# ERGO-Code/ipx

Measured on AMD Instinct MI355X. Metric: kkt_solves_per_sec, higher is better.
Workload: dtype f64; 1 GPU; C3 synthetic LP m=1000000 n=2000000 8 nnz/col (nnz=16000000), KKTSolverDiag::Solve = diag-precond CR to tol=0.3*sqrt(mu), scaling spread s=1; rows of AI partitioned over 1 GPU(s); errflag=0

## Files before the change

### ipx_amd/csrc/api.hip

```cpp

#include <algorithm>
#include <map>
#include <thread>

#include "context.hpp"

namespace ipxk {

static thread_local std::string g_last_error;
void set_last_error(const std::string& msg) { g_last_error = msg; }

Context::~Context() {
    if (split) destroy_split(split);
    if (split_spare) destroy_split(split_spare);
    if (prepare_host) destroy_prepare_host(prepare_host);
    if (lu) destroy_lu(lu);
    if (maxvol) destroy_maxvol(maxvol);
    if (nmat) destroy_nmatrix(nmat);
    comm_destroy(this);
    if (h_state) (void)hipHostFree(h_state);
    if (h_cycle_done) (void)hipHostFree(h_cycle_done);
    if (ev_a) (void)hipEventDestroy(ev_a);
    if (ev_b) (void)hipEventDestroy(ev_b);
    for (hipEvent_t e : ev_window) (void)hipEventDestroy(e);
// ... 1198 lines not shown
        IPXK_REQUIRE(c && info && (which == 0 || which == 1), "bad argument");
        const GatherMatrix& M = which == 0 ? c->Acols : c->Arows;
        for (int i = 0; i < 40; i++) info[i] = 0;
        const SpmvLayout L = M.layout;
        info[0] = M.tile_base() != SpmvLayout::phased; info[1] = L == SpmvLayout::sorted; info[2] = L == SpmvLayout::sortedfused; info[3] = M.nlong;
        info[4] = M.sliced.built; info[5] = M.sliced.R; info[6] = M.sliced.nslices; info[7] = M.sliced.nrb;
        info[8] = M.sliced.nrows_pad; info[9] = M.sliced.max_tile;
        { double d = M.sliced.dominant_fraction; memcpy(&info[10], &d, sizeof d); }
        info[11] = M.sorted.built; info[12] = M.sorted.nslices; info[13] = M.sorted.nsub; info[14] = M.sorted.nrb;
        info[15] = M.sorted.RB; info[16] = M.sorted.nrows_pad; info[17] = M.sorted.max_sub; info[18] = M.sorted.slice_elems;
        info[19] = M.sorted.fused; info[20] = M.nnz;
        info[21] = M.P; info[22] = M.G; info[23] = (ipxint)M.RT * 1000000 + (ipxint)M.Q * 1000 + 0;
        info[24] = L == SpmvLayout::acc; info[25] = M.acc.built; info[26] = M.acc.nslices; info[27] = M.acc.nrb; info[28] = M.acc.RB;
        info[29] = M.acc.nrows_pad; info[30] = M.acc.slice_elems; info[31] = M.acc.nbatches; info[32] = M.acc.deferred;
        info[33] = L == SpmvLayout::accfused; info[34] = M.accf.built; info[35] = M.accf.nrb; info[36] = M.accf.RB; info[37] = M.accf.nbatches;
        info[38] = L == SpmvLayout::plain;
        if (create_ms) for (int i = 0; i < 4; i++) create_ms[i] = c->create_ms[i];
    });
}
int ipxk_layout_array(ipxk_context* c, int which, int array, void* out, ipxint cap, ipxint* nbytes) {
    return guarded([&] {
        IPXK_REQUIRE(c && nbytes && (which == 0 || which == 1), "bad argument");
        bind_device(c);
        const GatherMatrix& M = which == 0 ? c->Acols : c->Arows;
        const void* src = nullptr;
        size_t bytes = 0;
        const size_t ntiles = (size_t)M.sliced.nrb * M.sliced.nslices, nsubs = (size_t)M.sorted.nrb * std::max(M.sorted.nslices, 1) * std::max(M.sorted.nsub, 1);
        const size_t nz = (size_t)M.nnz;
        switch (array) {
            case 0: src = M.sliced.tile_ptr.get(); bytes = M.sliced.built ? (ntiles + 1) * 4 : 0; break;
            case 1: src = M.sliced.cnt.get(); bytes = M.sliced.built ? ntiles * M.sliced.R : 0; break;
// ... 4 lines not shown
            case 6: src = M.sorted.pack.get(); bytes = M.sorted.built ? nz * 4 : 0; break;
            case 7: src = M.sorted.val.get(); bytes = M.sorted.built ? nz * 8 : 0; break;
            case 8: src = c->pl_Tp.get(); bytes = ((size_t)c->m + 1) * 4; break;
            case 9: src = c->pl_Ti.get(); bytes = (size_t)c->nnz * 4; break;
            case 10: src = c->pl_Tx.get(); bytes = (size_t)c->nnz * 8; break;
            case 11: src = M.acc.tile_batch.get(); bytes = M.acc.built ? ((size_t)M.acc.nrb * M.acc.nslices + 1) * 4 : 0; break;
            case 12: src = M.acc.bptr.get(); bytes = M.acc.built ? ((size_t)M.acc.nbatches + 1) * 4 : 0; break;
            case 13: src = M.acc.pack.get(); bytes = M.acc.built ? nz * 4 : 0; break;
            case 14: src = M.acc.val.get(); bytes = M.acc.built ? nz * 8 : 0; break;
            case 15: src = M.accf.tile_batch.get(); bytes = M.accf.built ? ((size_t)M.accf.nrb + 1) * 4 : 0; break;
            case 16: src = M.accf.bptr.get(); bytes = M.accf.built ? ((size_t)M.accf.nbatches + 1) * 4 : 0; break;
            case 17: src = M.accf.pack.get(); bytes = M.accf.built ? nz * 4 : 0; break;
            case 18: src = M.accf.val.get(); bytes = M.accf.built ? nz * 8 : 0; break;
            case 19: src = M.accf.xmin.get(); bytes = M.accf.built ? (size_t)M.accf.nrb * 4 : 0; break;
            case 20: src = M.sorted.xmin.get(); bytes = M.sorted.built && M.sorted.fused ? (size_t)M.sorted.nrb * 4 : 0; break;
            default: IPXK_REQUIRE(false, "unknown array");
        }
        if (M.nlong > 0 && (array < 8 || array > 10)) bytes = 0;
        *nbytes = (ipxint)bytes;
        const size_t ncopy = std::min<size_t>(bytes, cap > 0 ? (size_t)cap : 0);
        if (out && ncopy > 0) staged_d2h(out, src, ncopy, c->stream);
    });
}

ipxint ipxk_normal_apply_bytes(const ipxk_context* c) {
    if (!c) return 0;
    const ipxint wi = 4;
    return 2 * c->nnz * (wi + 8) + (c->n + c->m + 2) * wi + 8 * (3 * c->n + 4 * c->m);
}

// ... 50 lines not shown
```

### ipx_amd/csrc/context.hpp

```cpp
#pragma once

#include "internal.hpp"
#include "device_utils.hpp"

struct ncclComm;

namespace ipxk {

constexpr int kPartialStride = kMaxPartials + 8;

enum PartialSlot {
    kPartRes0 = 0,
    kPartRes1,
    kPartPdot,
    kPartCdot,
    kPartRsdot,
    kPartScratch,
    kNumPartialSlots
};

struct Reordered {
    bool active = false;
    int levels = 0;
    int components = 0;
// ... 136 lines not shown
void device_transpose(Tmp& T, DevBuf<int>& colof, int64_t n, int64_t m, int64_t nz, const int* Ap, const int* Ai, const double* Ax, int* Tp,
                      int* Ti, double* Tx, hipStream_t s);

bool device_strip_long_rows(LayoutScratch& S, GatherMatrix& G, int nrows, const int* dptr, const int* didx, const double* dval,
                            DevBuf<int>& sptr, DevBuf<int>& sidx, DevBuf<double>& sval, int64_t* nnz_short, hipStream_t s);
bool device_build_sliced(LayoutScratch& S, SlicedMatrix& out, int nrows, int ncols, int64_t nnz, const int* dptr, const int* didx,
                         const double* dval, hipStream_t s, int ns_request = 0);
bool device_build_sorted_fused(LayoutScratch& S, SortedMatrix& out, int nrows, int ncols, int64_t nnz, const int* dptr, const int* didx,
                               const double* dval, hipStream_t s);
bool device_build_acc_fused(LayoutScratch& S, AccMatrix& out, int nrows, int ncols, int64_t nnz, const int* dptr, const int* didx,
                            const double* dval, hipStream_t s);
bool device_build_sorted(LayoutScratch& S, SortedMatrix& out, const SlicedMatrix& sliced, int nrows, int ncols, int64_t nnz, const int* dptr,
                         const int* didx, const double* dval, hipStream_t s);
bool device_build_acc(LayoutScratch& S, AccMatrix& out, const SlicedMatrix& sliced, int nrows, int ncols, int64_t nnz, const int* dptr,
                      const int* didx, const double* dval, hipStream_t s);

void reorder_model(Context* c);
void reorder_permute_rows(Context* c, const double* in_old, double* out_new);
void reorder_unpermute_rows(Context* c, const double* in_new, double* out_old);
void reorder_permute_weights(Context* c, const double* W_old, double* W_new);

void dense_lu_inverse(Context* c, int kb, const double* D, const double* invL, const double* invU, double* X, double* Xt, int refine = 0);

enum TimeKind { kTimeOp = 0, kTimePrecond = 1, kTimeB = 2, kTimeBt = 3, kNumTimeKinds = 4 };
void time_mark(Context* c, int kind, bool begin);
void time_start(Context* c, ipxk_times* times);
void time_collect(Context* c, ipxk_times* times);

const double* stage_in(Context* c, const double* p, size_t len, DevBuf<double>& buf);
double* stage_out(Context* c, double* p, size_t len, DevBuf<double>& buf);
// ... 199 lines not shown
```

### ipx_amd/csrc/internal.hpp

```cpp
#pragma once

#include <hip/hip_runtime.h>

#include <chrono>
#include <cstdint>
#include <cstdio>
#include <cstdlib>
#include <algorithm>
#include <cstring>
#include <functional>
#include <memory>
#include <stdexcept>
#include <string>
#include <type_traits>
#include <vector>

#include "../../include/ipx_kkt_hip.h"

namespace ipxk {

struct Error : std::runtime_error {
    int code;
    Error(int c, const std::string& what) : std::runtime_error(what), code(c) {}
};
// ... 146 lines not shown
};
struct SortedMatrix {
    bool built = false;
    int nslices = 0, nsub = 0, nrb = 0, RB = 0, nrows_pad = 0, max_sub = 0, slice_elems = 0;
    DevBuf<unsigned> sub_ptr, pack;
    DevBuf<unsigned char> cnt;
    DevBuf<double> val, partial;
    bool fused = false;
    DevBuf<int> xmin;
};

constexpr int kAccThreads = 512;
constexpr int kAccPerThread = 4;
constexpr int kAccBatch = kAccThreads * kAccPerThread;
constexpr int kAccMaxRows = 16384;
struct AccView {
    int nrows, nrows_pad, nslices, nrb, RB, slice_elems;
    const int* xmin;
    const unsigned* tile_batch;
    const unsigned* bptr;
    const unsigned* pack;
    const double* val;
    double* partial;
};
struct AccMatrix {
    bool built = false;
    int nslices = 0, nrb = 0, RB = 0, nrows_pad = 0, slice_elems = 0;
    int64_t nbatches = 0, deferred = 0;
    DevBuf<unsigned> tile_batch, bptr, pack;
    DevBuf<double> val, partial;
    bool fused = false;
    DevBuf<int> xmin;
};

struct LayoutScratch;

enum class SpmvLayout { phased, sliced, fused, sorted, sortedfused, acc, plain, accfused };
constexpr int kNumSpmvLayouts = 8;
inline constexpr const char* kSpmvLayoutNames[kNumSpmvLayouts] = {"phased", "sliced", "fused", "sorted", "sortedfused", "acc", "plain",
                                                                  "accfused"};

inline int combine_grid_for(int64_t nrows) {
    static const int cap = [] { const char* e = getenv("IPXK_COMBINE_GRID"); return e && atoi(e) > 0 ? std::min(atoi(e), 1024) : 1024; }();
    return (int)std::min<int64_t>(cap, std::max<int64_t>(1, (nrows + kBlock - 1) / kBlock));
// ... 207 lines not shown
```

### ipx_amd/csrc/layout_device.hip

```cpp
#include <numeric>
#include <rocprim/device/device_radix_sort.hpp>
#include <rocprim/device/device_scan.hpp>

#include "layout_scratch.hpp"

namespace ipxk {

template <class K>
void sort_pairs(Tmp& T, const K* kin, K* kout, const unsigned* vin, unsigned* vout, size_t n, int bits, hipStream_t s) {
    size_t bytes = 0;
    IPXK_HIP(rocprim::radix_sort_pairs(nullptr, bytes, kin, kout, vin, vout, n, 0u, (unsigned)bits, s));
    IPXK_HIP(rocprim::radix_sort_pairs(T.need(bytes), bytes, kin, kout, vin, vout, n, 0u, (unsigned)bits, s));
}
template void sort_pairs<unsigned>(Tmp&, const unsigned*, unsigned*, const unsigned*, unsigned*, size_t, int, hipStream_t);
template void sort_pairs<u64>(Tmp&, const u64*, u64*, const unsigned*, unsigned*, size_t, int, hipStream_t);
void sort_keys(Tmp& T, u64* in, u64* out, size_t n, hipStream_t s) {
    size_t bytes = 0;
    IPXK_HIP(rocprim::radix_sort_keys(nullptr, bytes, in, out, n, 0u, 64u, s));
    IPXK_HIP(rocprim::radix_sort_keys(T.need(bytes), bytes, in, out, n, 0u, 64u, s));
}
void scan_int(Tmp& T, const int* in, int* out, size_t n, hipStream_t s) {
    size_t bytes = 0;
    IPXK_HIP(rocprim::exclusive_scan(nullptr, bytes, in, out, 0, n, rocprim::plus<int>(), s));
    IPXK_HIP(rocprim::exclusive_scan(T.need(bytes), bytes, in, out, 0, n, rocprim::plus<int>(), s));
// ... 176 lines not shown
    IPXK_GRID_STRIDE(e, nz) {
        const unsigned d = dst[e];
        pack[d] = word[e];
        out_val[d] = val[perm[e]];
    }
}
__global__ void acc_bptr_kernel(int ntiles, const unsigned* __restrict__ tile_ptr, const unsigned* __restrict__ tile_batch,
                                const unsigned* __restrict__ bstart, unsigned nz, unsigned* __restrict__ bptr) {
    const int tile = blockIdx.x;
    if (tile >= ntiles) return;
    const unsigned e0 = tile_ptr[tile], b0 = tile_batch[tile], nb = tile_batch[tile + 1] - b0;
    for (unsigned q = threadIdx.x; q < nb; q += blockDim.x) bptr[b0 + q] = bstart[e0 + q];
    if (tile == ntiles - 1 && threadIdx.x == 0) bptr[tile_batch[ntiles]] = nz;
}

__global__ void tile_window_kernel(int nrows, const int* __restrict__ ptr, const int* __restrict__ idx, int RB, int* __restrict__ lo,
                                   int* __restrict__ hi, unsigned char* __restrict__ cnt, int* flags) {
    IPXK_GRID_STRIDE(r, nrows) {
        const int p0 = ptr[r], p1 = ptr[r + 1];
        if (cnt) { if (p1 - p0 > 255) flags[0] = 1; cnt[r] = (unsigned char)(p1 - p0); }
        if (p1 == p0) continue;
        int a = idx[p0], b = a;
        for (int p = p0 + 1; p < p1; p++) {
            const int v = idx[p];
            if (v <= idx[p - 1]) flags[1] = 1;
            a = min(a, v); b = max(b, v);
        }
        atomicMin(lo + r / RB, a);
        atomicMax(hi + r / RB, b);
    }
// ... 246 lines not shown
int acc_rows_per_block(int nrows, int ns) {
    static const int cap = [] { const char* e = getenv("IPXK_ACC_ROWS"); return e && atoi(e) >= 1024 ? std::min(atoi(e), kAccMaxRows) & ~1 : kAccMaxRows; }();
    static const bool balance = !(getenv("IPXK_ACC_BALANCE") && getenv("IPXK_ACC_BALANCE")[0] == '0');
    if (const int G = balance ? acc_persist_grid(ns) : 0) {
        const int64_t per = G / ns;
        const int64_t nrb = (((int64_t)nrows + cap - 1) / cap + per - 1) / per * per;
        int rb = (int)(((int64_t)nrows + nrb - 1) / nrb);
        rb += rb & 1;
        if (rb >= 1024 && 8 * (int64_t)rb >= 7 * (int64_t)cap) return rb;
    }
    int RB = cap;
    while (RB > 1024 && ((int64_t)nrows + RB - 1) / RB * (int64_t)ns < 256) RB /= 2;
    return RB;
}

struct AccTemps {
    DevBuf<int> rowof;
    DevBuf<unsigned> tile_ptr, nbatch, bstart;
    AccTemps(int64_t ntiles, size_t nz) : rowof(nz), tile_ptr((size_t)ntiles + 1), nbatch((size_t)ntiles + 1), bstart(nz) {}
};
static void acc_batches(LayoutScratch& S, AccMatrix& out, AccTemps& T, int64_t ntiles, int RB, int64_t nnz, const double* dval, hipStream_t s) {
    const size_t nz = (size_t)nnz;
    unsigned* word = S.k1.get();
    hipLaunchKernelGGL(acc_words_kernel, dim3(gridn(nnz)), dim3(kBlock), 0, s, nnz, S.q2.get(), S.v2.get(), T.rowof.get(), RB, word);
    IPXK_HIP(hipMemsetAsync(S.stats.get(), 0, 8 * sizeof(int), s));
    const size_t lds = (size_t)RB * 2 * sizeof(unsigned);
    IPXK_HIP(hipFuncSetAttribute(reinterpret_cast<const void*>(acc_batch_kernel), hipFuncAttributeMaxDynamicSharedMemorySize,
                                 (int)(kAccMaxRows * 2 * sizeof(unsigned))));
    hipLaunchKernelGGL(acc_batch_kernel, dim3((unsigned)ntiles), dim3(64), lds, s, RB, T.tile_ptr.get(), word, S.k2.get(), S.v3.get(), S.v4.get(),
                       T.bstart.get(), T.nbatch.get(), reinterpret_cast<u64*>(S.stats.get()));
    out.tile_batch.ensure((size_t)ntiles + 1);
    scan_u32((int)ntiles, T.nbatch.get(), out.tile_batch.get(), s);
    unsigned nb_total = 0;
    u64 ndef = 0;
    IPXK_HIP(hipMemcpyAsync(&nb_total, out.tile_batch.get() + ntiles, sizeof(unsigned), hipMemcpyDeviceToHost, s));
    IPXK_HIP(hipMemcpyAsync(&ndef, S.stats.get(), sizeof(u64), hipMemcpyDeviceToHost, s));
    IPXK_HIP(hipStreamSynchronize(s));
    out.bptr.ensure((size_t)nb_total + 1); out.pack.ensure(nz); out.val.ensure(nz);
    hipLaunchKernelGGL(acc_bptr_kernel, dim3((unsigned)ntiles), dim3(64), 0, s, (int)ntiles, T.tile_ptr.get(), out.tile_batch.get(), T.bstart.get(),
                       (unsigned)nnz, out.bptr.get());
    hipLaunchKernelGGL(acc_scatter_kernel, dim3(gridn(nnz)), dim3(kBlock), 0, s, nnz, S.k2.get(), word, S.v2.get(), dval, out.pack.get(),
                       out.val.get());
    out.nbatches = nb_total; out.deferred = (int64_t)ndef;
}

static void tile_windows(LayoutScratch& S, int nrows, int nrb, int RB, const int* dptr, const int* didx, int* lo, int* hi, unsigned char* cnt,
                         int h[4], hipStream_t s) {
    IPXK_HIP(hipMemsetAsync(lo, 0x7f, (size_t)nrb * sizeof(int), s));
    IPXK_HIP(hipMemsetAsync(hi, 0xff, (size_t)nrb * sizeof(int), s));
    if (cnt) IPXK_HIP(hipMemsetAsync(cnt, 0, (size_t)nrb * RB, s));
    IPXK_HIP(hipMemsetAsync(S.stats.get(), 0, 8 * sizeof(int), s));
    hipLaunchKernelGGL(tile_window_kernel, dim3(gridn(nrows)), dim3(kBlock), 0, s, nrows, dptr, didx, RB, lo, hi, cnt, S.stats.get() + 2);
    hipLaunchKernelGGL(tile_window_stats_kernel, dim3(gridn(nrb)), dim3(kBlock), 0, s, nrb, nrows, RB, dptr, lo, hi, S.stats.get());
    IPXK_HIP(hipMemcpyAsync(h, S.stats.get(), 4 * sizeof(int), hipMemcpyDeviceToHost, s));
    IPXK_HIP(hipStreamSynchronize(s));
}

bool device_build_acc(LayoutScratch& S, AccMatrix& out, const SlicedMatrix& sliced, int nrows, int ncols, int64_t nnz, const int* dptr,
// ... 90 lines not shown
```

### ipx_amd/csrc/layout_host.hip

```cpp
#include <algorithm>
#include <cstdio>
#include <cstdlib>
#include <utility>

#include "context.hpp"

namespace ipxk {

void GatherMatrix::build(int64_t nrows_, int64_t ncols_, const ipxint* hptr, const ipxint* hidx,
                         const double* hval, hipStream_t s) {
    IPXK_REQUIRE(nrows_ >= 0 && ncols_ >= 0, "negative dimension");
    IPXK_REQUIRE(nrows_ < (int64_t(1) << 31) - 1 && ncols_ < (int64_t(1) << 31) - 1,
                 "dimension exceeds 32-bit device indices");
    const int64_t nz = hptr[nrows_];
    IPXK_REQUIRE(nz < (int64_t(1) << 31) - kLongSeg, "nnz exceeds 32-bit device indices");
    nrows = (int)nrows_;
    ncols = (int)ncols_;
    nnz = nz;

    set_geometry(nrows_, ncols_);
    const int64_t slice = phase_slice(ncols_);
    const int64_t RW = (int64_t)kBlock * RT;
    const int64_t nsteps = (int64_t)Q * P * G;
    IPXK_REQUIRE(nsteps * RW < (int64_t(1) << 40), "matrix too large for the phased layout");
// ... 311 lines not shown
            };
            for (int i : pend) offer(i);
            while (fill < kAccBatch && cursor < ne) offer(cursor++);
            pend.swap(newpend);
            batch++;
        }
    }
    void finish(AccMatrix& A, std::vector<unsigned>& tb, int64_t nnz, hipStream_t s) {
        tb.back() = (unsigned)bp.size();
        bp.push_back((unsigned)nnz);
        A.nbatches = (int64_t)bp.size() - 1; A.deferred = deferred;
        A.tile_batch.upload(tb, s);
        A.bptr.upload(bp, s);
        A.pack.upload(pk, s);
        A.val.upload(tv, s);
    }
};
}

void GatherMatrix::build_acc(const ipxint* hptr, const ipxint* hidx, const double* hval, hipStream_t s) {
    acc = AccMatrix();
    if (!sliced.built || sliced.nslices < 2 || nlong > 0 || nnz == 0) return;
    const int ns = sliced.nslices;
    const int64_t slice = slice_width(ncols, ns);
    if (!offsets_fit(slice)) return;
    const int RB = acc_rows_per_block(nrows, ns);
    const int nrb = (nrows + RB - 1) / RB;
    const int64_t ntiles = (int64_t)nrb * ns;
    std::vector<unsigned> tptr((size_t)ntiles + 1, 0);
    for (int r = 0; r < nrows; r++)
// ... 130 lines not shown
```

### ipx_amd/csrc/nmatrix.hip

```cpp
#include "layout_scratch.hpp"
#include "spmv_kernels.hpp"
#include "trisolve.hpp"

namespace ipxk {

namespace {

constexpr int kTileShift = 42, kRowShift = 32;

__global__ void nm_keep_kernel(int n, const double* __restrict__ W, const int* __restrict__ Ap, int* __restrict__ keep, int* __restrict__ len) {
    IPXK_GRID_STRIDE(j, n) {
        const int k = W[j] != 0.0 ? 1 : 0;
        keep[j] = k;
        len[j] = k ? Ap[j + 1] - Ap[j] : 0;
    }
}
__global__ void nm_colof_kernel(int n, const int* __restrict__ keep, const int* __restrict__ newidx, int* __restrict__ colof,
                                int* __restrict__ newidx_or_minus) {
    IPXK_GRID_STRIDE(j, n) {
        if (keep[j]) colof[newidx[j]] = (int)j;
        newidx_or_minus[j] = keep[j] ? newidx[j] : -1;
    }
}
__global__ void nm_diff_kernel(int n, const int* __restrict__ keep, const int* __restrict__ keep_prev, int* out) {
// ... 253 lines not shown
static void launch_tiles(const SlicedMatrix& P, int nrows, const double* x, const Epi& epi, const int* done, hipStream_t s) {
    const SlicedView V = view_of(P, nrows);
    const size_t lds = (size_t)(P.max_tile + P.max_tile / 32 + 1) * sizeof(double);
    const dim3 grid(V.nrb * V.nslices), block(kBlock);
    if (V.R == kBlock * 4) hipLaunchKernelGGL((spmv_sliced_tile_kernel<Epi, 4, false, false>), grid, block, lds, s, V, x, epi, (double*)nullptr, done);
    else if (V.R == kBlock * 2) hipLaunchKernelGGL((spmv_sliced_tile_kernel<Epi, 2, false, false>), grid, block, lds, s, V, x, epi, (double*)nullptr, done);
    else hipLaunchKernelGGL((spmv_sliced_tile_kernel<Epi, 1, false, false>), grid, block, lds, s, V, x, epi, (double*)nullptr, done);
    launch_combine(V, epi, (double*)nullptr, done, s);
}

template <class Epi>
static void launch_acc(const AccMatrix& A, const SlicedMatrix& P, int nrows, const double* x, const Epi& epi, const int* done, hipStream_t s) {
    AccView W;
    W.nrows = nrows; W.nrows_pad = A.nrows_pad; W.nslices = A.nslices; W.nrb = A.nrb; W.RB = A.RB; W.slice_elems = A.slice_elems;
    W.tile_batch = A.tile_batch.get(); W.bptr = A.bptr.get(); W.pack = A.pack.get(); W.val = A.val.get(); W.partial = A.partial.get();
    launch_acc_tiles<Epi>(W, x, done, s);
    SlicedView V = view_of(P, nrows);
    V.nrows_pad = A.nrows_pad; V.partial = A.partial.get();
    launch_combine(V, epi, (double*)nullptr, done, s);
}

void nmatrix_apply(Context* c, const double* WI, const double* u, double* work, const int* done) {
    NMatrix& N = *c->nmat;
    hipStream_t s = c->stream;
    EpiScale e1{{}, N.wN.get(), N.tN.get()};
    EpiNormalRows e2{{}, WI, u, work};
    if (N.A1.built && N.A2.built) {
        launch_acc(N.A1, N.P1, N.nN, u, e1, done, s);
        launch_acc(N.A2, N.P2, (int)c->m, N.tN.get(), e2, done, s);
        return;
// ... 7 lines not shown
```

### ipx_amd/csrc/spmv.hip

```cpp
#include <algorithm>
#include <cstdio>
#include <cstdlib>
#include <string>
#include <utility>

#include "context.hpp"
#include "spmv_kernels.hpp"

namespace ipxk {

int slice_elems() {
    static int cached = 0;
    if (!cached) {
        int kb = 1024;
        if (const char* e = getenv("IPXK_SLICE_KB")) kb = atoi(e) > 0 ? atoi(e) : kb;
        cached = kb * 128;
    }
    return cached;
}

int64_t phase_slice(int64_t ncols_) {
    constexpr int kMaxPhases = 64;
    int64_t slice = slice_elems();
    if ((ncols_ + slice - 1) / slice > kMaxPhases) slice = (ncols_ + kMaxPhases - 1) / kMaxPhases;
// ... 106 lines not shown
        if (tune_level > 1 && !env_off("IPXK_SPMV_SORTED")) consider(L::sortedfused);
        if (tune_level > 1 && !env_off("IPXK_SPMV_ACC")) consider(L::accfused);
        if (layout != L::accfused && nnz <= (int64_t(4) << 20) && !env_off("IPXK_SPMV_PLAIN")) consider(L::plain);
    }
    if (sliced.built) {
        idx.release(); val.release(); counts.release(); step_ptr.release();
        wg_chunk_ptr.release(); chunk_start.release(); chunk_info.release(); chunk_step.release();
    }
    if (getenv("IPXK_VERBOSE")) {
        fprintf(stderr, "ipxk: gather matrix %d x %d nnz %lld:", nrows, ncols, (long long)nnz);
        for (int l = 0; l < kNumSpmvLayouts; l++)
            if (tuned_us[l] > 0.f) fprintf(stderr, " %s %.1f us,", kSpmvLayoutNames[l], tuned_us[l]);
        fprintf(stderr, " fullest-slice share %.2f -> %s\n", share, kSpmvLayoutNames[(int)layout]);
        const AccMatrix& a = layout == L::accfused ? accf : acc;
        if (a.built)
            fprintf(stderr, "ipxk:   %d rows per tile, %lld batches, %.1f%% of the entries waited\n", a.RB, (long long)a.nbatches,
                    100.0 * (double)a.deferred / (double)nnz);
    }
}

bool GatherMatrix::build_device_local(LayoutScratch& S, int64_t nrows_, int64_t ncols_, int64_t nnz_, const int* dptr, const int* didx,
                                      const double* dval, double share, hipStream_t s) {
    if (getenv("IPXK_LAYOUT_LOCAL") && getenv("IPXK_LAYOUT_LOCAL")[0] == 'h') return false;
    SlicedMatrix fu;
    if (!device_build_sliced(S, fu, (int)nrows_, (int)ncols_, nnz_, dptr, didx, dval, s, 1)) return false;
    nrows = (int)nrows_; ncols = (int)ncols_; nnz = nnz_;
    set_geometry(nrows_, ncols_);
    fu.dominant_fraction = share;
    select_layout([&](SpmvLayout L) {
        switch (L) {
            case SpmvLayout::fused: sliced = std::move(fu); return true;
            case SpmvLayout::sortedfused: {
// ... 58 lines not shown
                sorted = std::move(so);
                return true;
            }
            default: return false;
        }
    }, s);
    nnz = nnz_all;
    return true;
}

static AccView view_of(const AccMatrix& A, int nrows) {
    AccView V;
    V.nrows = nrows; V.nrows_pad = A.nrows_pad; V.nslices = A.nslices; V.nrb = A.nrb; V.RB = A.RB; V.slice_elems = A.slice_elems;
    V.xmin = A.xmin.get();
    V.tile_batch = A.tile_batch.get(); V.bptr = A.bptr.get(); V.pack = A.pack.get(); V.val = A.val.get(); V.partial = A.partial.get();
    return V;
}
AccView GatherMatrix::acc_view() const { return view_of(acc, nrows); }
AccView GatherMatrix::acc_fused_view() const { return view_of(accf, nrows); }

SortedView GatherMatrix::sorted_view() const {
    SortedView V;
    V.xmin = sorted.fused ? sorted.xmin.get() : nullptr;
    V.row_long = sorted.fused && nlong > 0 ? row_long.get() : nullptr;
    V.nrows = nrows; V.nrows_pad = sorted.nrows_pad; V.nslices = sorted.nslices; V.nsub = sorted.nsub; V.nrb = sorted.nrb;
    V.RB = sorted.RB; V.slice_elems = sorted.slice_elems;
    V.sub_ptr = sorted.sub_ptr.get(); V.cnt = sorted.cnt.get(); V.pack = sorted.pack.get(); V.val = sorted.val.get();
    V.partial = sorted.partial.get();
    return V;
}
// ... 111 lines not shown
```

### ipx_amd/csrc/spmv_kernels.hpp

```cpp
#pragma once

#include <type_traits>

#include "device_utils.hpp"
#include "internal.hpp"

namespace ipxk {

constexpr int kLdsDoubles = kChunkNnz + kChunkNnz / 32;

__device__ __forceinline__ int lds_slot(int q) { return q + (q >> 5); }

template <class Epi, class = void>
struct EpiRow {
    struct In {};
    static __device__ __forceinline__ In load(const Epi&, long long) { return In{}; }
    static __device__ __forceinline__ double init(const Epi& e, long long r, const In&) { return e.init((int)r); }
    static __device__ __forceinline__ void finish(const Epi& e, long long r, const In&, double acc, double& dot) { e.finish((int)r, acc, dot); }
};
template <class Epi>
struct EpiRow<Epi, std::void_t<typename Epi::In>> {
    using In = typename Epi::In;
    static __device__ __forceinline__ In load(const Epi& e, long long r) { return e.load(r); }
    static __device__ __forceinline__ double init(const Epi& e, long long, const In& in) { return e.init(in); }
// ... 645 lines not shown
                stream(pk[d % 3], v[d % 3], e[3], e[4]);
#pragma unroll
                for (int i = 0; i + 1 < NE; i++) e[i] = e[i + 1];
                e[NE - 1] = enew;
            }
        }
    }
    __syncthreads();
    double* dst = M.partial + (size_t)s * M.nrows_pad + (size_t)rb * M.RB;
    for (int r = 2 * tid; r < M.RB; r += 2 * T) reinterpret_cast<double2*>(dst + r)[0] = make_double2(ac_sum[r], ac_sum[r + 1]);
}

constexpr int kAccParkPairs = kAccMaxRows / (2 * kAccThreads);
constexpr int kAccParkPerBatch = 2;
template <class Prod>
__global__ __launch_bounds__(kAccThreads) void spmv_acc_persist_kernel(AccView M, const unsigned* __restrict__ tile_batch,
                                                                       const unsigned* __restrict__ bptr, const double* __restrict__ x,
                                                                       const int* done) {
    const int dn = *(done ? done : reinterpret_cast<const int*>(tile_batch));
    extern __shared__ double ac_sum[];
    constexpr int U = kAccPerThread, T = kAccThreads, NP = kAccParkPairs, PB = kAccParkPerBatch;
    static_assert(NP % PB == 0, "parked pairs per batch");
    const int tid = threadIdx.x;
    const int ntiles = M.nrb * M.nslices, G = gridDim.x;
    const int s = blockIdx.x % M.nslices;
    const double* __restrict__ xs = x + (size_t)s * M.slice_elems;
    double* const part = M.partial + (size_t)s * M.nrows_pad;
    struct Batch { unsigned e0, e1; int tile; };
    int wt = blockIdx.x, wq = 0, wnb = 0;
    unsigned wb0 = 0;
    if (wt < ntiles) { wb0 = tile_batch[wt]; wnb = (int)(tile_batch[wt + 1] - wb0); }
    if (done && dn) return;
    auto next = [&]() -> Batch {
        Batch b{0u, 0u, -1};
        if (wt >= ntiles) return b;
        b.tile = wt;
        if (wnb > 0) { b.e0 = bptr[wb0 + wq]; b.e1 = bptr[wb0 + wq + 1]; }
        if (++wq >= max(wnb, 1)) {
            wt += G; wq = 0;
            if (wt < ntiles) { wb0 = tile_batch[wt]; wnb = (int)(tile_batch[wt + 1] - wb0); }
        }
        return b;
    };
    constexpr int NE = 6;
    Batch q[NE];
#pragma unroll
    for (int i = 0; i < NE; i++) q[i] = next();
    unsigned pk[3][U];
    double v[3][U], xg[2][U];
    auto stream = [&](unsigned (&pkb)[U], double (&vb)[U], unsigned e0, unsigned e1) {
        const int ne = (int)(e1 - e0);
        const unsigned base = ne > 0 ? e0 : 0u;
        const int last = max(ne - 1, 0);
#pragma unroll
        for (int u = 0; u < U; u++) {
            const int i = min(u * T + tid, last);
            pkb[u] = __builtin_nontemporal_load(M.pack + base + i);
            vb[u] = __builtin_nontemporal_load(M.val + base + i);
        }
    };
    auto gather = [&](double (&xgb)[U], const unsigned (&pkb)[U], const Batch& b) {
        const bool live = b.e1 > b.e0;
        const double* __restrict__ xb = live ? xs : x;
        const unsigned mask = live ? (1u << kSortedOffBits) - 1u : 0u;
#pragma unroll
        for (int u = 0; u < U; u++) xgb[u] = xb[pkb[u] & mask];
    };
#pragma unroll
    for (int d = 0; d < 3; d++) {
#pragma unroll
        for (int u = 0; u < U; u++) { pk[d][u] = 0u; v[d][u] = 0.0; }
        stream(pk[d], v[d], q[d].e0, q[d].e1);
    }
    for (int r = tid; r < M.RB; r += T) ac_sum[r] = 0.0;
    gather(xg[0], pk[0], q[0]);
    int cur = q[0].tile;
// ... 23 lines not shown
#pragma unroll
                    for (int j = 0; j < NP; j++) {
                        const int r = 2 * tid + 2 * T * j;
                        if (r < M.RB) {
                            park[j] = make_double2(ac_sum[r], ac_sum[r + 1]);
                            ac_sum[r] = 0.0;
                            ac_sum[r + 1] = 0.0;
                        }
                    }
                    pdst = part + (size_t)(cur / M.nslices) * M.RB;
                    prow = 2 * tid;
                    pleft = NP / PB;
                    cur = q[0].tile;
                    __syncthreads();
                }
#pragma unroll
                for (int u = 0; u < U; u++)
                    if (u * T + tid < ne)
                        __hip_atomic_fetch_add(ac_sum + (pk[d % 3][u] >> kSortedOffBits), Prod::prod(xg[d & 1][u], v[d % 3][u]), __ATOMIC_RELAXED,
                                               __HIP_MEMORY_SCOPE_WORKGROUP);
                stream(pk[d % 3], v[d % 3], q[3].e0, q[3].e1);
                if (pleft > 0) store_parked();
#pragma unroll
                for (int i = 0; i + 1 < NE; i++) q[i] = q[i + 1];
                q[NE - 1] = next();
            }
        }
    }
    __syncthreads();
    while (pleft > 0) store_parked();
    if (cur >= 0) {
        double* dst = part + (size_t)(cur / M.nslices) * M.RB;
        for (int r = 2 * tid; r < M.RB; r += 2 * T) reinterpret_cast<double2*>(dst + r)[0] = make_double2(ac_sum[r], ac_sum[r + 1]);
    }
}
// ... 218 lines not shown
    else launch_combine_ns<Epi, false>(V, epi, dot_partials, done, s);
}

template <class Prod>
inline void launch_acc_tiles(const AccView& W, const double* x, const int* done, hipStream_t s) {
    static bool lds_attr_set = false;
    if (!lds_attr_set) {
        IPXK_HIP(hipFuncSetAttribute(reinterpret_cast<const void*>(spmv_acc_tile_kernel<Prod>), hipFuncAttributeMaxDynamicSharedMemorySize,
                                     (int)(kAccMaxRows * sizeof(double))));
        IPXK_HIP(hipFuncSetAttribute(reinterpret_cast<const void*>(spmv_acc_persist_kernel<Prod>), hipFuncAttributeMaxDynamicSharedMemorySize,
                                     (int)(kAccMaxRows * sizeof(double))));
        lds_attr_set = true;
    }
    const size_t lds = (size_t)W.RB * sizeof(double);
    const int ntiles = W.nrb * W.nslices, G = acc_persist_grid(W.nslices);
    if (G > 0) hipLaunchKernelGGL((spmv_acc_persist_kernel<Prod>), dim3(std::min(G, ntiles)), dim3(kAccThreads), lds, s, W, W.tile_batch, W.bptr,
                                  x, done);
    else hipLaunchKernelGGL((spmv_acc_tile_kernel<Prod>), dim3(ntiles), dim3(kAccThreads), lds, s, W, x, done);
}

template <class Epi, bool MASKED = false, bool COMPACT = false>
inline void launch_spmv_sliced(const GatherMatrix& M, const double* x, const Epi& epi, double* dot_partials,
                               const int* done, hipStream_t s) {
    static_assert(!(MASKED && COMPACT), "the compacted copy needs no mask");
    const SlicedView V = M.sliced_view(COMPACT ? 2 : MASKED ? 1 : 0);
    const size_t lds = (size_t)(M.sliced.max_tile + M.sliced.max_tile / 32 + 1) * sizeof(double);
    const dim3 grid(V.nrb * V.nslices), block(kBlock);
    if (V.nslices == 1) {
        const dim3 fgrid(M.fused_grid());
        if (V.R == kBlock * 4) hipLaunchKernelGGL((spmv_sliced_tile_kernel<Epi, 4, true, MASKED>), fgrid, block, lds, s, V, x, epi, dot_partials, done);
        else if (V.R == kBlock * 2) hipLaunchKernelGGL((spmv_sliced_tile_kernel<Epi, 2, true, MASKED>), fgrid, block, lds, s, V, x, epi, dot_partials, done);
// ... 79 lines not shown
```

### ipx_amd/kkt.py

```python
import ctypes as C
import os
import subprocess

import numpy as np

HERE = os.path.dirname(os.path.abspath(__file__))
LIB_PATH = os.path.join(HERE, "lib", "libipx_kkt_hip.so")

i64, f64 = np.int64, np.float64
c_i64, c_f64 = C.c_int64, C.c_double
P_i64, P_f64 = C.POINTER(C.c_int64), C.POINTER(C.c_double)
INTERRUPT_FN = C.CFUNCTYPE(c_i64, C.c_void_p)

POINTER_HOST, POINTER_DEVICE = 0, 1
NONBASIC_FIXED, NONBASIC, BASIC, BASIC_FREE = -2, -1, 0, 1

EXPORTS = [
    "ipxk_last_error", "ipxk_device_count", "ipxk_create", "ipxk_destroy", "ipxk_set_pointer_mode",
    "ipxk_set_stream", "ipxk_synchronize", "ipxk_set_profiling", "ipxk_set_interrupt", "ipxk_reset_solver_state", "ipxk_get_reorder_info", "ipxk_get_reordering", "ipxk_num_dense_cols", "ipxk_get_rowwise",
    "ipxk_normal_prepare", "ipxk_normal_apply", "ipxk_diag_factorize", "ipxk_diag_apply",
    "ipxk_diag_get", "ipxk_pcr_solve", "ipxk_cr_diagnostics", "ipxk_kkt_diag_factorize", "ipxk_kkt_diag_solve",
    "ipxk_kkt_diag_get", "ipxk_split_prepare", "ipxk_split_rescale", "ipxk_split_apply", "ipxk_forward_solve",
    "ipxk_backward_solve", "ipxk_solve_dense", "ipxk_split_levels", "ipxk_cr_solve",
    "ipxk_kkt_basis_solve", "ipxk_newton_solve", "ipxk_iterate_set", "ipxk_iterate_get", "ipxk_iterate_update",
# ... 282 lines not shown
        a, b, w = C.c_int64(0), C.c_int64(0), C.c_double(0.0)
        self._check(self.lib.ipxk_split_inverse_stats(self.h, C.byref(a), C.byref(b), C.byref(w)))
        return a.value, b.value, w.value

    def split_inverse_refined(self):
        return int(self.lib.ipxk_split_inverse_refined(self.h))

    def layout_info(self, which):
        info = (C.c_int64 * 40)()
        ms = (C.c_double * 4)()
        self._check(self.lib.ipxk_layout_info(self.h, which, info, ms))
        keys = ("use_sliced", "use_sorted", "use_sorted_fused", "nlong", "sliced_built", "R", "nslices", "nrb", "nrows_pad",
                "max_tile", "dominant_bits", "sorted_built", "so_nslices", "so_nsub", "so_nrb", "so_RB", "so_nrows_pad",
                "so_max_sub", "so_slice_elems", "so_fused", "nnz", "P", "G", "RTQ", "use_acc", "acc_built", "acc_nslices", "acc_nrb",
                "acc_RB", "acc_nrows_pad", "acc_slice_elems", "acc_nbatches", "acc_deferred", "use_acc_fused", "accf_built", "accf_nrb", "accf_RB",
                "accf_nbatches", "use_plain")
        d = {k: int(v) for k, v in zip(keys, info)}
        d["dominant_fraction"] = float(np.array([d.pop("dominant_bits")], dtype=np.int64).view(np.float64)[0])
        return d, [float(v) for v in ms]

    def layout_array(self, which, array):
        dt = (np.uint32, np.uint8, np.int32, np.float64, np.uint32, np.uint8, np.uint32, np.float64, np.int32, np.int32, np.float64,
              np.uint32, np.uint32, np.uint32, np.float64, np.uint32, np.uint32, np.uint32, np.float64, np.int32, np.int32)[array]
        nb = C.c_int64(0)
        self._check(self.lib.ipxk_layout_array(self.h, which, array, None, 0, C.byref(nb)))
        out = np.zeros(nb.value // np.dtype(dt).itemsize, dtype=dt)
        if nb.value:
            self._check(self.lib.ipxk_layout_array(self.h, which, array, out.ctypes.data_as(C.c_void_p), nb.value, C.byref(nb)))
            self._check(self.lib.ipxk_synchronize(self.h))
        return out

    def get_rowwise(self):
        nnz = int(self._keep[0][-1])
        p, i, x = np.zeros(self.m + 1, i64), np.zeros(nnz, i64), np.zeros(nnz, f64)
        self._check(self.lib.ipxk_get_rowwise(self.h, _ip(p), _ip(i), _fp(x)))
        return p, i, x

    def normal_prepare(self, W):
# ... 464 lines not shown
```

Baseline: 59.93 solves/s.

## Merge up to four small accumulation batches into one step in persistent SpMV

Adds a precomputed per-tile step table that packs up to four consecutive conflict-free batches (total size within one batch width) into a single uint4 step record. The persistent acc SpMV kernel now streams and gathers one step at a time and applies the sub-batches in order, separated by __syncthreads, so small batches no longer each pay a full pipeline slot. This is meant to reduce per-batch loads and gathers that carried little work. In exchange, the layout build gains extra kernels plus a host sync, and the kernel gains a branchy inner loop with extra barriers.

```diff
diff --git a/ipx_amd/csrc/api.hip b/ipx_amd/csrc/api.hip
--- a/ipx_amd/csrc/api.hip
+++ b/ipx_amd/csrc/api.hip
@@ -1236,7 +1236,7 @@
         info[24] = L == SpmvLayout::acc; info[25] = M.acc.built; info[26] = M.acc.nslices; info[27] = M.acc.nrb; info[28] = M.acc.RB;
         info[29] = M.acc.nrows_pad; info[30] = M.acc.slice_elems; info[31] = M.acc.nbatches; info[32] = M.acc.deferred;
         info[33] = L == SpmvLayout::accfused; info[34] = M.accf.built; info[35] = M.accf.nrb; info[36] = M.accf.RB; info[37] = M.accf.nbatches;
-        info[38] = L == SpmvLayout::plain;
+        info[38] = L == SpmvLayout::plain; info[39] = M.acc.nsteps;
         if (create_ms) for (int i = 0; i < 4; i++) create_ms[i] = c->create_ms[i];
     });
 }
@@ -1271,6 +1271,8 @@
             case 18: src = M.accf.val.get(); bytes = M.accf.built ? nz * 8 : 0; break;
             case 19: src = M.accf.xmin.get(); bytes = M.accf.built ? (size_t)M.accf.nrb * 4 : 0; break;
             case 20: src = M.sorted.xmin.get(); bytes = M.sorted.built && M.sorted.fused ? (size_t)M.sorted.nrb * 4 : 0; break;
+            case 21: src = M.acc.tile_step.get(); bytes = M.acc.built ? ((size_t)M.acc.nrb * M.acc.nslices + 1) * 4 : 0; break;
+            case 22: src = M.acc.steps.get(); bytes = M.acc.built ? ((size_t)M.acc.nsteps + 1) * 16 : 0; break;
             default: IPXK_REQUIRE(false, "unknown array");
         }
         if (M.nlong > 0 && (array < 8 || array > 10)) bytes = 0;
diff --git a/ipx_amd/csrc/context.hpp b/ipx_amd/csrc/context.hpp
--- a/ipx_amd/csrc/context.hpp
+++ b/ipx_amd/csrc/context.hpp
@@ -174,6 +174,7 @@
                          const int* didx, const double* dval, hipStream_t s);
 bool device_build_acc(LayoutScratch& S, AccMatrix& out, const SlicedMatrix& sliced, int nrows, int ncols, int64_t nnz, const int* dptr,
                       const int* didx, const double* dval, hipStream_t s);
+void acc_build_steps(AccMatrix& A, int64_t ntiles, int64_t nnz, hipStream_t s);
 
 void reorder_model(Context* c);
 void reorder_permute_rows(Context* c, const double* in_old, double* out_new);
diff --git a/ipx_amd/csrc/internal.hpp b/ipx_amd/csrc/internal.hpp
--- a/ipx_amd/csrc/internal.hpp
+++ b/ipx_amd/csrc/internal.hpp
@@ -184,11 +184,14 @@
 constexpr int kAccPerThread = 4;
 constexpr int kAccBatch = kAccThreads * kAccPerThread;
 constexpr int kAccMaxRows = 16384;
+constexpr int kAccStepBatches = 4;
 struct AccView {
     int nrows, nrows_pad, nslices, nrb, RB, slice_elems;
     const int* xmin;
     const unsigned* tile_batch;
     const unsigned* bptr;
+    const unsigned* tile_step;
+    const uint4* steps;
     const unsigned* pack;
     const double* val;
     double* partial;
@@ -196,8 +199,9 @@
 struct AccMatrix {
     bool built = false;
     int nslices = 0, nrb = 0, RB = 0, nrows_pad = 0, slice_elems = 0;
-    int64_t nbatches = 0, deferred = 0;
-    DevBuf<unsigned> tile_batch, bptr, pack;
+    int64_t nbatches = 0, deferred = 0, nsteps = 0;
+    DevBuf<unsigned> tile_batch, bptr, pack, tile_step;
+    DevBuf<uint4> steps;
     DevBuf<double> val, partial;
     bool fused = false;
     DevBuf<int> xmin;
diff --git a/ipx_amd/csrc/layout_device.hip b/ipx_amd/csrc/layout_device.hip
--- a/ipx_amd/csrc/layout_device.hip
+++ b/ipx_amd/csrc/layout_device.hip
@@ -214,6 +214,33 @@
     if (tile == ntiles - 1 && threadIdx.x == 0) bptr[tile_batch[ntiles]] = nz;
 }
 
+template <class Emit>
+__device__ __forceinline__ unsigned acc_tile_steps(const unsigned* __restrict__ bptr, unsigned b0, unsigned b1, unsigned maxb, Emit emit) {
+    unsigned ns = 0;
+    for (unsigned b = b0; b < b1; ns++) {
+        unsigned k = 1;
+        while (k < maxb && b + k < b1 && bptr[b + k + 1] - bptr[b] <= (unsigned)kAccBatch) k++;
+        emit(ns, b, k);
+        b += k;
+    }
+    return ns;
+}
+__global__ void acc_step_count_kernel(int ntiles, const unsigned* __restrict__ tile_batch, const unsigned* __restrict__ bptr, unsigned maxb,
+                                      unsigned* __restrict__ nstep) {
+    IPXK_GRID_STRIDE(t, ntiles) nstep[t] = acc_tile_steps(bptr, tile_batch[t], tile_batch[t + 1], maxb, [](unsigned, unsigned, unsigned) {});
+}
+__global__ void acc_step_fill_kernel(int ntiles, const unsigned* __restrict__ tile_batch, const unsigned* __restrict__ bptr, unsigned maxb,
+                                     const unsigned* __restrict__ tile_step, unsigned nz, uint4* __restrict__ steps) {
+    IPXK_GRID_STRIDE(t, ntiles) {
+        const unsigned s0 = tile_step[t];
+        acc_tile_steps(bptr, tile_batch[t], tile_batch[t + 1], maxb, [&](unsigned i, unsigned b, unsigned k) {
+            const unsigned end = bptr[b + k];
+            steps[s0 + i] = make_uint4(bptr[b], k > 1 ? bptr[b + 1] : end, k > 2 ? bptr[b + 2] : end, k > 3 ? bptr[b + 3] : end);
+        });
+        if (t == ntiles - 1) steps[tile_step[ntiles]] = make_uint4(nz, nz, nz, nz);
+    }
+}
+
 __global__ void tile_window_kernel(int nrows, const int* __restrict__ ptr, const int* __restrict__ idx, int RB, int* __restrict__ lo,
                                    int* __restrict__ hi, unsigned char* __restrict__ cnt, int* flags) {
     IPXK_GRID_STRIDE(r, nrows) {
@@ -490,6 +517,24 @@
     return RB;
 }
 
+void acc_build_steps(AccMatrix& A, int64_t ntiles, int64_t nnz, hipStream_t s) {
+    static const bool merge = !(getenv("IPXK_ACC_STEPS") && getenv("IPXK_ACC_STEPS")[0] == '0');
+    static_assert(kAccStepBatches == 4, "a step record holds three cuts");
+    const unsigned maxb = merge ? kAccStepBatches : 1;
+    DevBuf<unsigned> nstep((size_t)ntiles + 1);
+    hipLaunchKernelGGL(acc_step_count_kernel, dim3(gridn(ntiles)), dim3(kBlock), 0, s, (int)ntiles, A.tile_batch.get(), A.bptr.get(), maxb, nstep.get());
+    A.tile_step.ensure((size_t)ntiles + 1);
+    scan_u32((int)ntiles, nstep.get(), A.tile_step.get(), s);
+    unsigned total = 0;
+    IPXK_HIP(hipMemcpyAsync(&total, A.tile_step.get() + ntiles, sizeof(unsigned), hipMemcpyDeviceToHost, s));
+    IPXK_HIP(hipStreamSynchronize(s));
+    A.steps.ensure((size_t)total + 1);
+    hipLaunchKernelGGL(acc_step_fill_kernel, dim3(gridn(ntiles)), dim3(kBlock), 0, s, (int)ntiles, A.tile_batch.get(), A.bptr.get(), maxb,
+                       A.tile_step.get(), (unsigned)nnz, A.steps.get());
+    IPXK_HIP(hipStreamSynchronize(s));
+    A.nsteps = total;
+}
+
 struct AccTemps {
     DevBuf<int> rowof;
     DevBuf<unsigned> tile_ptr, nbatch, bstart;
@@ -518,6 +563,7 @@
     hipLaunchKernelGGL(acc_scatter_kernel, dim3(gridn(nnz)), dim3(kBlock), 0, s, nnz, S.k2.get(), word, S.v2.get(), dval, out.pack.get(),
                        out.val.get());
     out.nbatches = nb_total; out.deferred = (int64_t)ndef;
+    acc_build_steps(out, ntiles, nnz, s);
 }
 
 static void tile_windows(LayoutScratch& S, int nrows, int nrb, int RB, const int* dptr, const int* didx, int* lo, int* hi, unsigned char* cnt,
diff --git a/ipx_amd/csrc/layout_host.hip b/ipx_amd/csrc/layout_host.hip
--- a/ipx_amd/csrc/layout_host.hip
+++ b/ipx_amd/csrc/layout_host.hip
@@ -349,6 +349,7 @@
         A.bptr.upload(bp, s);
         A.pack.upload(pk, s);
         A.val.upload(tv, s);
+        acc_build_steps(A, (int64_t)tb.size() - 1, nnz, s);
     }
 };
 }
diff --git a/ipx_amd/csrc/nmatrix.hip b/ipx_amd/csrc/nmatrix.hip
--- a/ipx_amd/csrc/nmatrix.hip
+++ b/ipx_amd/csrc/nmatrix.hip
@@ -291,6 +291,7 @@
     AccView W;
     W.nrows = nrows; W.nrows_pad = A.nrows_pad; W.nslices = A.nslices; W.nrb = A.nrb; W.RB = A.RB; W.slice_elems = A.slice_elems;
     W.tile_batch = A.tile_batch.get(); W.bptr = A.bptr.get(); W.pack = A.pack.get(); W.val = A.val.get(); W.partial = A.partial.get();
+    W.tile_step = A.tile_step.get(); W.steps = A.steps.get();
     launch_acc_tiles<Epi>(W, x, done, s);
     SlicedView V = view_of(P, nrows);
     V.nrows_pad = A.nrows_pad; V.partial = A.partial.get();
diff --git a/ipx_amd/csrc/spmv.hip b/ipx_amd/csrc/spmv.hip
--- a/ipx_amd/csrc/spmv.hip
+++ b/ipx_amd/csrc/spmv.hip
@@ -144,8 +144,8 @@
         fprintf(stderr, " fullest-slice share %.2f -> %s\n", share, kSpmvLayoutNames[(int)layout]);
         const AccMatrix& a = layout == L::accfused ? accf : acc;
         if (a.built)
-            fprintf(stderr, "ipxk:   %d rows per tile, %lld batches, %.1f%% of the entries waited\n", a.RB, (long long)a.nbatches,
-                    100.0 * (double)a.deferred / (double)nnz);
+            fprintf(stderr, "ipxk:   %d rows per tile, %lld steps / %lld batches, %.1f%% of the entries waited\n", a.RB, (long long)a.nsteps,
+                    (long long)a.nbatches, 100.0 * (double)a.deferred / (double)nnz);
     }
 }
 
@@ -234,6 +234,7 @@
     V.nrows = nrows; V.nrows_pad = A.nrows_pad; V.nslices = A.nslices; V.nrb = A.nrb; V.RB = A.RB; V.slice_elems = A.slice_elems;
     V.xmin = A.xmin.get();
     V.tile_batch = A.tile_batch.get(); V.bptr = A.bptr.get(); V.pack = A.pack.get(); V.val = A.val.get(); V.partial = A.partial.get();
+    V.tile_step = A.tile_step.get(); V.steps = A.steps.get();
     return V;
 }
 AccView GatherMatrix::acc_view() const { return view_of(acc, nrows); }
diff --git a/ipx_amd/csrc/spmv_kernels.hpp b/ipx_amd/csrc/spmv_kernels.hpp
--- a/ipx_amd/csrc/spmv_kernels.hpp
+++ b/ipx_amd/csrc/spmv_kernels.hpp
@@ -683,10 +683,10 @@
 constexpr int kAccParkPairs = kAccMaxRows / (2 * kAccThreads);
 constexpr int kAccParkPerBatch = 2;
 template <class Prod>
-__global__ __launch_bounds__(kAccThreads) void spmv_acc_persist_kernel(AccView M, const unsigned* __restrict__ tile_batch,
-                                                                       const unsigned* __restrict__ bptr, const double* __restrict__ x,
+__global__ __launch_bounds__(kAccThreads) void spmv_acc_persist_kernel(AccView M, const unsigned* __restrict__ tile_step,
+                                                                       const uint4* __restrict__ steps, const double* __restrict__ x,
                                                                        const int* done) {
-    const int dn = *(done ? done : reinterpret_cast<const int*>(tile_batch));
+    const int dn = *(done ? done : reinterpret_cast<const int*>(tile_step));
     extern __shared__ double ac_sum[];
     constexpr int U = kAccPerThread, T = kAccThreads, NP = kAccParkPairs, PB = kAccParkPerBatch;
     static_assert(NP % PB == 0, "parked pairs per batch");
@@ -695,24 +695,27 @@
     const int s = blockIdx.x % M.nslices;
     const double* __restrict__ xs = x + (size_t)s * M.slice_elems;
     double* const part = M.partial + (size_t)s * M.nrows_pad;
-    struct Batch { unsigned e0, e1; int tile; };
+    struct Step { unsigned e0, e1, c1, c2, c3; int tile; };
     int wt = blockIdx.x, wq = 0, wnb = 0;
     unsigned wb0 = 0;
-    if (wt < ntiles) { wb0 = tile_batch[wt]; wnb = (int)(tile_batch[wt + 1] - wb0); }
+    if (wt < ntiles) { wb0 = tile_step[wt]; wnb = (int)(tile_step[wt + 1] - wb0); }
     if (done && dn) return;
-    auto next = [&]() -> Batch {
-        Batch b{0u, 0u, -1};
+    auto next = [&]() -> Step {
+        Step b{0u, 0u, 0u, 0u, 0u, -1};
         if (wt >= ntiles) return b;
         b.tile = wt;
-        if (wnb > 0) { b.e0 = bptr[wb0 + wq]; b.e1 = bptr[wb0 + wq + 1]; }
+        if (wnb > 0) {
+            const uint4 r = steps[wb0 + wq];
+            b.e0 = r.x; b.c1 = r.y; b.c2 = r.z; b.c3 = r.w; b.e1 = steps[wb0 + wq + 1].x;
+        }
         if (++wq >= max(wnb, 1)) {
             wt += G; wq = 0;
-            if (wt < ntiles) { wb0 = tile_batch[wt]; wnb = (int)(tile_batch[wt + 1] - wb0); }
+            if (wt < ntiles) { wb0 = tile_step[wt]; wnb = (int)(tile_step[wt + 1] - wb0); }
         }
         return b;
     };
     constexpr int NE = 6;
-    Batch q[NE];
+    Step q[NE];
 #pragma unroll
     for (int i = 0; i < NE; i++) q[i] = next();
     unsigned pk[3][U];
@@ -728,7 +731,7 @@
             vb[u] = __builtin_nontemporal_load(M.val + base + i);
         }
     };
-    auto gather = [&](double (&xgb)[U], const unsigned (&pkb)[U], const Batch& b) {
+    auto gather = [&](double (&xgb)[U], const unsigned (&pkb)[U], const Step& b) {
         const bool live = b.e1 > b.e0;
         const double* __restrict__ xb = live ? xs : x;
         const unsigned mask = live ? (1u << kSortedOffBits) - 1u : 0u;
@@ -782,11 +785,25 @@
                     cur = q[0].tile;
                     __syncthreads();
                 }
+                const int n1 = (int)(q[0].c1 - q[0].e0);
 #pragma unroll
                 for (int u = 0; u < U; u++)
-                    if (u * T + tid < ne)
+                    if (u * T + tid < n1)
                         __hip_atomic_fetch_add(ac_sum + (pk[d % 3][u] >> kSortedOffBits), Prod::prod(xg[d & 1][u], v[d % 3][u]), __ATOMIC_RELAXED,
                                                __HIP_MEMORY_SCOPE_WORKGROUP);
+                if (n1 < ne) {
+                    int lo = n1, hi = (int)(q[0].c2 - q[0].e0), hi2 = (int)(q[0].c3 - q[0].e0);
+#pragma unroll 1
+                    for (int p = 1; p < kAccStepBatches && lo < ne; p++) {
+                        __syncthreads();
+#pragma unroll
+                        for (int u = 0; u < U; u++)
+                            if (u * T + tid >= lo && u * T + tid < hi)
+                                __hip_atomic_fetch_add(ac_sum + (pk[d % 3][u] >> kSortedOffBits), Prod::prod(xg[d & 1][u], v[d % 3][u]),
+                                                       __ATOMIC_RELAXED, __HIP_MEMORY_SCOPE_WORKGROUP);
+                        lo = hi; hi = hi2; hi2 = ne;
+                    }
+                }
                 stream(pk[d % 3], v[d % 3], q[3].e0, q[3].e1);
                 if (pleft > 0) store_parked();
 #pragma unroll
@@ -1035,7 +1052,7 @@
     }
     const size_t lds = (size_t)W.RB * sizeof(double);
     const int ntiles = W.nrb * W.nslices, G = acc_persist_grid(W.nslices);
-    if (G > 0) hipLaunchKernelGGL((spmv_acc_persist_kernel<Prod>), dim3(std::min(G, ntiles)), dim3(kAccThreads), lds, s, W, W.tile_batch, W.bptr,
+    if (G > 0) hipLaunchKernelGGL((spmv_acc_persist_kernel<Prod>), dim3(std::min(G, ntiles)), dim3(kAccThreads), lds, s, W, W.tile_step, W.steps,
                                   x, done);
     else hipLaunchKernelGGL((spmv_acc_tile_kernel<Prod>), dim3(ntiles), dim3(kAccThreads), lds, s, W, x, done);
 }
diff --git a/ipx_amd/kkt.py b/ipx_amd/kkt.py
--- a/ipx_amd/kkt.py
+++ b/ipx_amd/kkt.py
@@ -320,14 +320,15 @@
                 "max_tile", "dominant_bits", "sorted_built", "so_nslices", "so_nsub", "so_nrb", "so_RB", "so_nrows_pad",
                 "so_max_sub", "so_slice_elems", "so_fused", "nnz", "P", "G", "RTQ", "use_acc", "acc_built", "acc_nslices", "acc_nrb",
                 "acc_RB", "acc_nrows_pad", "acc_slice_elems", "acc_nbatches", "acc_deferred", "use_acc_fused", "accf_built", "accf_nrb", "accf_RB",
-                "accf_nbatches", "use_plain")
+                "accf_nbatches", "use_plain", "acc_nsteps")
         d = {k: int(v) for k, v in zip(keys, info)}
         d["dominant_fraction"] = float(np.array([d.pop("dominant_bits")], dtype=np.int64).view(np.float64)[0])
         return d, [float(v) for v in ms]
 
     def layout_array(self, which, array):
         dt = (np.uint32, np.uint8, np.int32, np.float64, np.uint32, np.uint8, np.uint32, np.float64, np.int32, np.int32, np.float64,
-              np.uint32, np.uint32, np.uint32, np.float64, np.uint32, np.uint32, np.uint32, np.float64, np.int32, np.int32)[array]
+              np.uint32, np.uint32, np.uint32, np.float64, np.uint32, np.uint32, np.uint32, np.float64, np.int32, np.int32,
+              np.uint32, np.uint32)[array]
         nb = C.c_int64(0)
         self._check(self.lib.ipxk_layout_array(self.h, which, array, None, 0, C.byref(nb)))
         out = np.zeros(nb.value // np.dtype(dt).itemsize, dtype=dt)
```

Measured after the change: 61.44 solves/s (median of 6 runs). +2.5%, better.
